# dusk-network/plonk_gadgets

Measured on AMD Instinct MI355X. Metric: gadget constraints/sec (range_check 256-bit), higher is better.
Workload: dtype u64x4 (BLS12-381 scalar, Montgomery limbs); 1 GPU; C2: 2^20 witnesses/GPU x (allocate + range_check(min=0,max=2^254)), n=255, 1031 rows + 1034 vars per witness; items_per_gpu=1048576, items_per_launch=1048576

## Files before the change

plonk_gadgets_amd/csrc/capi.hip:

```cpp
#include "../../include/plonk_gadgets_hip.h"

#include <hip/hip_runtime.h>

#include <algorithm>
#include <cstdio>
#include <cstdlib>
#include <cstring>
#include <initializer_list>
#include <new>
#include <functional>
#include <string>
#include <type_traits>
#include <utility>
#include <vector>

#include "emit.hpp"
#include "fr.hpp"
#include "range_gadgets.hpp"
#include "scalar_gadgets.hpp"
#include "composer.hpp"
#include "permutation.hpp"
#include "materialize.hpp"
#include "permutation_product.hpp"
#include "ntt.hpp"
// ... 17 lines not shown

#define PG_HIP_TRY(expr)                                                                \
    do {                                                                                \
        hipError_t _e = (expr);                                                         \
        if (_e != hipSuccess)                                                           \
            return fail(PG_ERR_HIP, std::string(#expr) + ": " + hipGetErrorString(_e)); \
    } while (0)

#define PG_TRY(expr)                   \
    do {                               \
        pg_status _s = (expr);         \
        if (_s != PG_OK) return _s;    \
    } while (0)

inline pg::Fr to_fr(const pg_scalar *s) {
    pg::Fr f;
    std::memcpy(f.l, s->l, sizeof f.l);
    return f;
}
inline void from_fr(const pg::Fr &f, pg_scalar *out) { std::memcpy(out->l, f.l, sizeof f.l); }

inline bool aligned(const void *p, size_t a) { return (reinterpret_cast<uintptr_t>(p) & (a - 1)) == 0; }

bool is_reduced(const pg::Fr &f) {
    const uint64_t Q[4] = {PG_Q0, PG_Q1, PG_Q2, PG_Q3};
    for (int i = 3; i >= 0; i--) {
        if (f.l[i] < Q[i]) return true;
        if (f.l[i] > Q[i]) return false;
    }
    return false;
}

pg_status check_columns(const pg_columns *c) {
    if (!c) return fail(PG_ERR_INVALID_ARGUMENT, "columns is NULL");
    const void *sc[6] = {c->q_m, c->q_l, c->q_r, c->q_o, c->q_c, c->var_values};
    for (const void *p : sc)
        if (!p || !aligned(p, 16)) return fail(PG_ERR_INVALID_ARGUMENT, "scalar column NULL or not 16-byte aligned");
    const void *wc[3] = {c->w_l, c->w_r, c->w_o};
    for (const void *p : wc)
        if (!p || !aligned(p, 8)) return fail(PG_ERR_INVALID_ARGUMENT, "wire column NULL or not 8-byte aligned");
    return PG_OK;
}

pg_status check_scalars(const void *p, const char *what) {
    if (!p || !aligned(p, 16)) return fail(PG_ERR_INVALID_ARGUMENT, std::string(what) + " NULL or not 16-byte aligned");
    return PG_OK;
}
pg_status check_u64s(const void *p, const char *what, bool nullable = false) {
    if (!p && nullable) return PG_OK;
    if (!p || !aligned(p, 8)) return fail(PG_ERR_INVALID_ARGUMENT, std::string(what) + " NULL or not 8-byte aligned");
    return PG_OK;
}

}

struct pg_engine {
    int device = -1;
    int num_cus = 0;
    uint4 *d_pow2 = nullptr;
    uint32_t *d_rows = nullptr, *d_vars = nullptr;
    uint64_t *d_blk_rows = nullptr, *d_blk_vars = nullptr;
    unsigned long long *d_blk_agg = nullptr;
    uint32_t *d_err_count = nullptr;
    uint64_t scratch_items = 0, scratch_blocks = 0;
    using PlanResult = pg::PlanTotals;
    PlanResult *h_plan = nullptr;
    uint4 *d_prefix = nullptr;
    uint64_t inv_elems = 0;
    hipStream_t side = nullptr;
    hipEvent_t ev_fork = nullptr, ev_inv = nullptr;
    hipStream_t last_stream = nullptr;
    bool have_last = false;
    hipEvent_t ev_switch = nullptr;
    uint4 *d_pp = nullptr;
    uint64_t pp_units = 0;
    uint4 *d_ntt = nullptr;
    uint64_t ntt_units = 0;
    uint4 *d_quot = nullptr, *d_eval = nullptr;
    uint64_t quot_units = 0, eval_units = 0;
    uint4 *d_msm = nullptr, *d_srs = nullptr;
    uint64_t msm_units = 0, srs_units = 0;
    uint4 *d_open = nullptr;
    uint64_t open_units = 0;
};

namespace {

pg_status ensure_scratch(pg_engine *e, uint64_t batch) {
    if (batch <= e->scratch_items && e->d_err_count) return PG_OK;
    PG_HIP_TRY(hipSetDevice(e->device));
    if (e->d_rows) { (void)hipFree(e->d_rows); e->d_rows = nullptr; }
    if (e->d_vars) { (void)hipFree(e->d_vars); e->d_vars = nullptr; }
    if (e->d_blk_rows) { (void)hipFree(e->d_blk_rows); e->d_blk_rows = nullptr; }
    if (e->d_blk_vars) { (void)hipFree(e->d_blk_vars); e->d_blk_vars = nullptr; }
    if (e->d_blk_agg) { (void)hipFree(e->d_blk_agg); e->d_blk_agg = nullptr; }
    e->scratch_items = 0;
    const uint64_t items = batch < 1024 ? 1024 : batch;
    const uint64_t nblk = std::max<uint64_t>((items + pg::kScanBlock - 1) / pg::kScanBlock, 2048);
    PG_HIP_TRY(hipMalloc(&e->d_rows, items * sizeof(uint32_t)));
    PG_HIP_TRY(hipMalloc(&e->d_vars, items * sizeof(uint32_t)));
    PG_HIP_TRY(hipMalloc(&e->d_blk_rows, nblk * sizeof(uint64_t)));
    PG_HIP_TRY(hipMalloc(&e->d_blk_vars, nblk * sizeof(uint64_t)));
    PG_HIP_TRY(hipMalloc(&e->d_blk_agg, (nblk + 1) * sizeof(unsigned long long)));
    PG_HIP_TRY(hipMemset(e->d_blk_agg, 0, (nblk + 1) * sizeof(unsigned long long)));
    e->scratch_blocks = nblk;
    if (!e->d_err_count) {
        PG_HIP_TRY(hipMalloc(&e->d_err_count, sizeof(uint32_t)));
        PG_HIP_TRY(hipMemset(e->d_err_count, 0, sizeof(uint32_t)));
    }
    e->scratch_items = items;
    return PG_OK;
}

pg::PlanScan plan_scan(pg_engine *e, uint64_t batch, uint64_t *d_row_off, uint64_t *d_var_off, bool with_errs) {
    const uint64_t nblk = (batch + pg::kScanBlock - 1) / pg::kScanBlock;
    pg::PlanScan P{};
    P.agg = e->d_blk_agg;
    P.blocks_cap = (uint32_t)e->scratch_blocks;
    P.blk_rows = e->d_blk_rows;
    P.blk_vars = e->d_blk_vars;
    P.row_off = d_row_off;
    P.var_off = d_var_off;
    P.host = e->h_plan;
    P.err_count = with_errs ? e->d_err_count : nullptr;
#if defined(PG_PLAN_TWO_LAUNCHES)
    P.fused = 0;
#else
    P.fused = nblk <= pg::kPlanFusedBlocks ? 1u : 0u;
#endif
    return P;
}

pg_status plan_totals(pg_engine *e, uint64_t *n_rows, uint64_t *n_vars) {
    if (e->h_plan->pad) {
        e->h_plan->pad = 0;
        return fail(PG_ERR_HIP, "a plan's look-back gave up waiting for another block's totals");
    }
    *n_rows = e->h_plan->n_gates;
    *n_vars = e->h_plan->n_vars;
    return PG_OK;
}

pg_status scan_counts(pg_engine *e, uint64_t batch, uint64_t *d_row_off, uint64_t *d_var_off, uint64_t *n_rows,
                      uint64_t *n_vars, hipStream_t st, bool with_errs) {
    const uint32_t nblk = (uint32_t)((batch + pg::kScanBlock - 1) / pg::kScanBlock);
    if (!plan_scan(e, batch, d_row_off, d_var_off, with_errs).fused) {
        const uint32_t prefixed = nblk > pg::kScanDirectBlocks ? 1u : 0u;
        if (prefixed)
            hipLaunchKernelGGL(pg::scan_top_kernel, dim3(1), dim3(pg::kThreads), 0, st, e->d_blk_rows, e->d_blk_vars, nblk);
        hipLaunchKernelGGL(pg::scan_final_kernel, dim3(nblk), dim3(pg::kThreads), 0, st, e->d_rows, e->d_vars, batch,
                           e->d_blk_rows, e->d_blk_vars, d_row_off, d_var_off, prefixed, e->h_plan, with_errs ? e->d_err_count : nullptr);
        PG_HIP_TRY(hipGetLastError());
    }
    if (n_rows) {
        PG_HIP_TRY(hipStreamSynchronize(st));
        PG_TRY(plan_totals(e, n_rows, n_vars));
    }
    return PG_OK;
}

pg::EmitOut make_out(const pg_columns *c, uint64_t batch, int W, uint64_t gate_base, uint64_t var_base, uint64_t zero_var,
                     const uint64_t *row_off, const uint64_t *var_off) {
    pg::EmitOut O;
    O.q[0] = reinterpret_cast<uint4 *>(c->q_m);
    O.q[1] = reinterpret_cast<uint4 *>(c->q_l);
    O.q[2] = reinterpret_cast<uint4 *>(c->q_r);
// ... 1313 lines not shown
```

plonk_gadgets_amd/csrc/capi_composer.inc:

```

struct pg_composer {
    pg_engine *e = nullptr;
    hipStream_t stream = nullptr;
    uint64_t gate_cap = 0, var_cap = 0, n = 0, nvars = 0, zero_var = 0;
    pg::ComposerCols cols{};
    uint64_t *d_stage = nullptr;
    std::vector<uint64_t> pi_gate;
    std::vector<pg_scalar> pi_val;
    std::vector<pg::FourthWire> fourth;
    std::vector<pg::PermSeg> segs;
    void *perm_small = nullptr, *perm_big = nullptr, *val_ws = nullptr;
    void *perm_pieces = nullptr;
    size_t perm_pieces_bytes = 0;
    size_t perm_small_bytes = 0, perm_big_bytes = 0, val_ws_bytes = 0;
    std::vector<void *> ragged;
    uint64_t *h_total = nullptr;
    uint64_t perm_last_sparse = 0;
    uint64_t sparse_hint = 0;
    uint64_t sparse_cap_first = 0;
    bool auto_grow = false;
    uint64_t col_stride = 0;
    void *block = nullptr;
    struct Queued {
        uint8_t kind;
// ... 1509 lines not shown
    const uint32_t grid = (uint32_t)c->e->num_cus * 32;
    pg::MaterializeOut M{};
    pg_scalar *const consts[7] = {out->q_4, out->q_arith, out->q_range, out->q_logic, out->q_fixed_group_add,
                                  out->q_variable_group_add, out->w_4_value};
    for (int k = 0; k < 7; k++) {
        if (!consts[k]) continue;
        PG_TRY(check_scalars(consts[k], "constant column"));
        M.konst[k] = reinterpret_cast<uint4 *>(consts[k]);
    }
    pg_scalar *const vals[3] = {out->w_l_value, out->w_r_value, out->w_o_value};
    for (int i = 0; i < 3; i++) {
        if (!vals[i]) continue;
        PG_TRY(check_scalars(vals[i], "wire value column"));
        M.val[i] = reinterpret_cast<uint4 *>(vals[i]);
    }
    if (out->w_4) {
        PG_TRY(check_u64s(out->w_4, "w_4"));
        M.w_4 = out->w_4;
    }
    const auto generic = [&](uint64_t lo, uint64_t hi) {
        if (hi <= lo) return;
        const uint64_t want = (2 * (hi - lo) + 16383) / 16384;
        hipLaunchKernelGGL(pg::materialize_kernel, dim3((uint32_t)(want < grid ? want : grid)), dim3(pg::kThreads), 0, c->stream, c->cols, M,
                           lo, hi, c->zero_var);
    };
    uint64_t at = 0;
    for (const pg::PermSeg &s : c->segs) {
        if (s.V > pg::kMatWindowVars || s.V == 0 || s.gate_end - s.gate_base < 4096) continue;
        generic(at, s.gate_base);
        uint64_t group = pg::kMatWindowVars / (s.V ? s.V : 1);
        group = group < 1 ? 1 : (group > s.items ? s.items : group);
#ifndef PG_MAT_GRID_PER_CU
#define PG_MAT_GRID_PER_CU 64
#endif
        const uint64_t n_groups = (s.items + group - 1) / group, most = (uint64_t)c->e->num_cus * PG_MAT_GRID_PER_CU;
        const dim3 mgrid((uint32_t)(n_groups < most ? n_groups : most));
        const bool closed = s.wire_kind != pg::WIRES_UNKNOWN && !s.row_off && (pg::ladder_foreign_per_item(s.wire_kind) == 0 || group <= pg::kMatWitItems);
#define PG_MAT_LAUNCH(MODE, KIND)                                                                                                          \
    hipLaunchKernelGGL((pg::materialize_items_kernel<MODE, KIND>), mgrid, dim3(pg::kMatThreads), 0, c->stream, c->cols, M, s, (uint32_t)group, \
                       c->zero_var)
        if (s.row_off && s.wire_kind == pg::WIRES_MAX_BOUND && group <= pg::kMatWitItems)
            hipLaunchKernelGGL((pg::materialize_items_kernel<pg::MAT_SELF, pg::WIRES_MAX_BOUND, true>), mgrid, dim3(pg::kMatThreads), 0, c->stream,
                               c->cols, M, s, (uint32_t)group, c->zero_var);
        else if (s.row_off && s.wire_kind == pg::WIRES_MIX && group < 127)
            hipLaunchKernelGGL((pg::materialize_items_kernel<pg::MAT_SELF, pg::WIRES_MIX, true>), mgrid, dim3(pg::kMatThreads), 0, c->stream,
                               c->cols, M, s, (uint32_t)group, c->zero_var);
        else if (!closed) PG_MAT_LAUNCH(pg::MAT_READ_WIRES, pg::WIRES_UNKNOWN);
        else if (s.wire_kind == pg::WIRES_RANGE_CHECK) PG_MAT_LAUNCH(pg::MAT_SELF, pg::WIRES_RANGE_CHECK);
        else if (s.wire_kind == pg::WIRES_MAX_BOUND) PG_MAT_LAUNCH(pg::MAT_SELF, pg::WIRES_MAX_BOUND);
        else if (s.wire_kind == pg::WIRES_RANGE_CHECK_ALLOCATED) PG_MAT_LAUNCH(pg::MAT_SELF, pg::WIRES_RANGE_CHECK_ALLOCATED);
        else if (s.wire_kind == pg::WIRES_MAX_BOUND_ALLOCATED) PG_MAT_LAUNCH(pg::MAT_SELF, pg::WIRES_MAX_BOUND_ALLOCATED);
        else if (s.wire_kind == pg::WIRES_DECOMPOSITION) PG_MAT_LAUNCH(pg::MAT_SELF, pg::WIRES_DECOMPOSITION);
        else if (s.wire_kind == pg::WIRES_MIX) PG_MAT_LAUNCH(pg::MAT_SELF, pg::WIRES_MIX);
        else PG_MAT_LAUNCH(pg::MAT_READ_WIRES, pg::WIRES_UNKNOWN);
#undef PG_MAT_LAUNCH
        at = s.gate_end;
    }
    generic(at, c->n);
    CallBuffers B(c->stream);
    uint64_t *d_gate; uint4 *d_val; pg::FourthWire *d_fw;
    PG_TRY(upload_sparse(c, B, &d_gate, &d_val, &d_fw));
    if (d_fw)
        hipLaunchKernelGGL(pg::patch_fourth_kernel, dim3(1), dim3(64), 0, c->stream, reinterpret_cast<uint4 *>(out->q_4), out->w_4,
                           reinterpret_cast<uint4 *>(out->w_4_value), c->cols.vars, d_fw, (uint32_t)c->fourth.size());
    PG_HIP_TRY(hipGetLastError());
    PG_HIP_TRY(hipStreamSynchronize(c->stream));
    return PG_OK;
}

#ifndef PG_PERM_LDS_PAD
#define PG_PERM_LDS_PAD 0
#endif
static pg_status perm_reserve(pg_composer *c, void **buf, size_t *have, size_t bytes) {
    if (bytes <= *have) return PG_OK;
    PG_HIP_TRY(hipStreamSynchronize(c->stream));
    if (*buf) (void)hipFree(*buf);
    *buf = nullptr;
    *have = 0;
    PG_HIP_TRY(hipMalloc(buf, bytes));
    *have = bytes;
    return PG_OK;
}

pg_status pg_composer_permutation_reserve(pg_composer *c, uint64_t sparse_positions) {
    if (!c) return fail(PG_ERR_INVALID_ARGUMENT, "composer is NULL");
    c->sparse_cap_first = sparse_positions;
    if (sparse_positions) c->perm_last_sparse = 0;
    return PG_OK;
}

pg_status pg_composer_permutation(pg_composer *c, uint64_t padded_n, uint64_t *d_sigma) {
    if (!c) return fail(PG_ERR_INVALID_ARGUMENT, "composer is NULL");
    PG_TRY(flush(c));
    PG_TRY(check_u64s(d_sigma, "d_sigma"));
    if (padded_n < c->n) return fail(PG_ERR_INVALID_ARGUMENT, "padded_n is smaller than the circuit");
    PG_HIP_TRY(hipSetDevice(c->e->device));
    const uint32_t grid = (uint32_t)c->e->num_cus * 32;
    if (!c->h_total) PG_HIP_TRY(hipHostMalloc(reinterpret_cast<void **>(&c->h_total), 32, hipHostMallocDefault));
    uint32_t pos_bits = 2, var_bits = 1;
    while ((1ull << pos_bits) < 4 * c->n) pos_bits++;
    while ((1ull << var_bits) < c->nvars + 1) var_bits++;
    if (pos_bits + var_bits > 64) return fail(PG_ERR_INVALID_ARGUMENT, "circuit too large for 64-bit (Variable, position) keys");
    std::vector<pg::PermSeg> segs;
    std::vector<std::pair<uint64_t, uint64_t>> gaps;
    uint64_t at = 0, gap_rows = 0;
    for (pg::PermSeg s : c->segs) {
        const auto fits = [&](uint64_t k) {
            return 4 * k * s.L < pg::kPermDone && k * s.V < pg::kPermNone &&
                   pg::perm_local_lds_bytes((uint32_t)(k * s.L), (uint32_t)(k * s.V)) <= pg::kPermLocalLdsLimit;
        };
        if (!fits(1)) continue;
        uint64_t k = 1024 / s.L;
        k = k < 1 ? 1 : (k > s.items ? s.items : k);
        while (k > 1 && !fits(k)) k--;
        const bool closed_ladder = s.wire_kind != pg::WIRES_UNKNOWN && s.wire_kind < pg::WIRES_MIX && (s.row_off ? s.wire_kind == pg::WIRES_MAX_BOUND && s.tail == 0 : s.wire_n >= 2);
        if (closed_ladder || (pg::is_template_kind(s.wire_kind) && s.tail == 0)) k = 1;
        s.group = (uint32_t)k;
        if (s.gate_base > at) gaps.emplace_back(at, s.gate_base);
        segs.push_back(s);
        at = s.gate_end;
    }
    if (c->n > at) gaps.emplace_back(at, c->n);
    for (const auto &g : gaps) gap_rows += g.second - g.first;
    const size_t seg_bytes = (segs.size() * sizeof(pg::PermSeg) + 255) / 256 * 256;
    const size_t fw_bytes = (c->fourth.size() * sizeof(pg::FourthWire) + 255) / 256 * 256;
    PG_TRY(perm_reserve(c, &c->perm_small, &c->perm_small_bytes, seg_bytes + fw_bytes + 256));
    char *small = static_cast<char *>(c->perm_small);
    pg::PermCtx X;
    X.C = c->cols; X.n = c->n; X.padded_n = padded_n; X.zero_var = c->zero_var;
    X.segs = reinterpret_cast<const pg::PermSeg *>(small); X.n_segs = (uint32_t)segs.size();
    X.fw = reinterpret_cast<const pg::FourthWire *>(small + seg_bytes); X.n_fw = (uint32_t)c->fourth.size();
    X.fw_lo = 0; X.fw_span = 0; X.pos_bits = pos_bits;
    X.hole_key = pos_bits + var_bits >= 64 ? ~0ull : (1ull << (pos_bits + var_bits)) - 1;
    if (!c->fourth.empty()) {
        uint64_t lo = ~0ull, hi = 0;
        for (const pg::FourthWire &f : c->fourth) { lo = f.gate < lo ? f.gate : lo; hi = f.gate > hi ? f.gate : hi; }
        X.fw_lo = lo; X.fw_span = hi - lo;
    }
    uint64_t reserved = 0;
    for (pg::PermSeg &s : segs)
        if (s.wire_kind != pg::WIRES_UNKNOWN && !s.row_off && s.wire_n >= 2) {
            s.sparse_base = reserved;
            reserved += s.items * pg::ladder_foreign_per_item(s.wire_kind);
        } else if (pg::is_template_kind(s.wire_kind) && s.tail == 0) {
            s.sparse_base = reserved;
            reserved += s.items * pg::template_foreign_per_item(s.wire_kind);
        }
    const auto ragged_ladder = [](const pg::PermSeg &s) { return s.row_off && s.wire_kind == pg::WIRES_MAX_BOUND && s.tail == 0; };
    const auto template_seg = [](const pg::PermSeg &s) { return pg::is_template_kind(s.wire_kind) && s.tail == 0; };
    const auto needs_pieces = [&](const pg::PermSeg &s) { return ragged_ladder(s) || (template_seg(s) && s.row_off); };
    const auto pieces_of = [](const pg::PermSeg &s) { return (s.gate_end - (s.gate_base & ~1ull) + pg::kPermLadderRows - 1) / pg::kPermLadderRows; };
    {
        uint64_t total_pieces = 0;
        for (const pg::PermSeg &s : segs)
            if (needs_pieces(s)) total_pieces += pieces_of(s);
        if (total_pieces) {
            PG_TRY(perm_reserve(c, &c->perm_pieces, &c->perm_pieces_bytes, total_pieces * sizeof(uint32_t)));
            uint32_t *at_piece = static_cast<uint32_t *>(c->perm_pieces);
            for (pg::PermSeg &s : segs)
                if (needs_pieces(s)) {
                    s.piece_item = at_piece;
                    at_piece += pieces_of(s);
                    const uint64_t want = (s.items + pg::kThreads - 1) / pg::kThreads;
                    hipLaunchKernelGGL(pg::perm_piece_items_kernel, dim3((uint32_t)(want < grid ? want : grid)), dim3(pg::kThreads), 0, c->stream, s,
                                       pg::kPermLadderRows, at_piece - pieces_of(s));
                }
            PG_HIP_TRY(hipGetLastError());
        }
    }
    unsigned long long *d_count = reinterpret_cast<unsigned long long *>(small + seg_bytes + fw_bytes);
    if (!segs.empty())
        PG_HIP_TRY(hipMemcpyAsync(small, segs.data(), segs.size() * sizeof(pg::PermSeg), hipMemcpyHostToDevice, c->stream));
    if (!c->fourth.empty())
        PG_HIP_TRY(hipMemcpyAsync(small + seg_bytes, c->fourth.data(), c->fourth.size() * sizeof(pg::FourthWire),
                                  hipMemcpyHostToDevice, c->stream));
    uint64_t cap = c->sparse_cap_first ? c->sparse_cap_first : 4 * gap_rows + c->sparse_hint + (1ull << 16), nS = 0;
    if (cap < c->perm_last_sparse) cap = c->perm_last_sparse;
    uint64_t *k0 = nullptr, *k1 = nullptr, holes = 0;
    size_t tmp_bytes = 0;
    for (int attempt = 0;; attempt++) {
        uint64_t *nul = nullptr;
        PG_HIP_TRY(rocprim::radix_sort_keys(nullptr, tmp_bytes, nul, nul, (size_t)cap, 0u, pos_bits + var_bits, c->stream));
        const size_t kb = (cap * 8 + 255) / 256 * 256;
        PG_TRY(perm_reserve(c, &c->perm_big, &c->perm_big_bytes, 2 * kb + tmp_bytes + 256));
        k0 = reinterpret_cast<uint64_t *>(c->perm_big);
        k1 = reinterpret_cast<uint64_t *>(static_cast<char *>(c->perm_big) + kb);
        const pg::PermSparse Q{k0, d_count, cap};
        hipLaunchKernelGGL(pg::perm_count_init_kernel, dim3(1), dim3(1), 0, c->stream, d_count, reserved);
        for (const pg::PermSeg &s : segs) {
            const uint64_t groups = (s.items + s.group - 1) / s.group, most = (uint64_t)c->e->num_cus * 64;
            if (s.wire_kind != pg::WIRES_UNKNOWN && !s.row_off && s.wire_n >= 2) {
                const uint64_t pieces = (s.gate_end - (s.gate_base & ~1ull) + pg::kPermLadderRows - 1) / pg::kPermLadderRows;
                const uint64_t lmost = pg::kPermLadderRows <= 2048 ? 0x7fffffffull : most;
                if (pg::kPermLadderLds)
                    PG_HIP_TRY(hipFuncSetAttribute(reinterpret_cast<const void *>(pg::perm_ladder_kernel<false>), hipFuncAttributeMaxDynamicSharedMemorySize,
                                                   (int)pg::kPermLadderLds));
                const uint32_t lds = pg::ladder_foreign_per_item(s.wire_kind) ? 0u : pg::kPermLadderLds;
                hipLaunchKernelGGL(pg::perm_ladder_kernel<false>, dim3((uint32_t)(pieces < lmost ? pieces : lmost)), dim3(pg::kThreads), lds,
                                   c->stream, X, s, Q, d_sigma);
                continue;
            }
            if (template_seg(s)) {
                const uint64_t pieces = pieces_of(s);
                if (pieces > 0x7fffffffull) return fail(PG_ERR_INVALID_ARGUMENT, "segment too large for one launch");
                const uint32_t lds = pg::template_foreign_per_item(s.wire_kind) ? 0u : pg::kPermLadderLds - 8192;
                const pg::TemplateRows T = pg::template_rows(s.wire_kind);
                if (s.row_off) {
                    PG_HIP_TRY(hipFuncSetAttribute(reinterpret_cast<const void *>(pg::perm_template_kernel<true>),
                                                   hipFuncAttributeMaxDynamicSharedMemorySize, (int)pg::kPermLadderLds));
                    hipLaunchKernelGGL(pg::perm_template_kernel<true>, dim3((uint32_t)pieces), dim3(pg::kThreads), lds, c->stream, X, s, T, Q, d_sigma);
                } else {
                    PG_HIP_TRY(hipFuncSetAttribute(reinterpret_cast<const void *>(pg::perm_template_kernel<false>),
                                                   hipFuncAttributeMaxDynamicSharedMemorySize, (int)pg::kPermLadderLds));
                    hipLaunchKernelGGL(pg::perm_template_kernel<false>, dim3((uint32_t)pieces), dim3(pg::kThreads), lds, c->stream, X, s, T, Q, d_sigma);
                }
                continue;
            }
            if (ragged_ladder(s)) {
                const uint64_t pieces = pieces_of(s);
                if (pieces > 0x7fffffffull) return fail(PG_ERR_INVALID_ARGUMENT, "segment too large for one launch");
                if (pg::kPermLadderLds)
                    PG_HIP_TRY(hipFuncSetAttribute(reinterpret_cast<const void *>(pg::perm_ladder_kernel<true>), hipFuncAttributeMaxDynamicSharedMemorySize,
                                                   (int)pg::kPermLadderLds));
                hipLaunchKernelGGL(pg::perm_ladder_kernel<true>, dim3((uint32_t)pieces), dim3(pg::kThreads), pg::kPermLadderLds, c->stream, X, s, Q,
                                   d_sigma);
                continue;
            }
            hipLaunchKernelGGL(pg::perm_item_kernel, dim3((uint32_t)(groups < most ? groups : most)), dim3(pg::kThreads),
                               pg::perm_local_lds_bytes(s.group * s.L, s.group * s.V) + PG_PERM_LDS_PAD, c->stream, X, s, groups, Q, d_sigma);
        }
        for (const auto &g : gaps) {
            const uint64_t nblk = (g.second - g.first + pg::kPermChunk - 1) / pg::kPermChunk;
            hipLaunchKernelGGL(pg::perm_gap_kernel, dim3((uint32_t)nblk), dim3(pg::kThreads), 0, c->stream, X, g.first, g.second, Q,
                               d_sigma);
        }
        PG_HIP_TRY(hipMemcpyAsync(c->h_total, d_count, 16, hipMemcpyDeviceToHost, c->stream));
        PG_HIP_TRY(hipStreamSynchronize(c->stream));
        nS = c->h_total[0];
        holes = c->h_total[1];
        c->perm_last_sparse = nS;
        if (nS <= cap) break;
        if (attempt) return fail(PG_ERR_HIP, "sparse position list grew between two passes");
        cap = nS;
    }
    if (nS) {
        PG_HIP_TRY(rocprim::radix_sort_keys(static_cast<char *>(c->perm_big) + 2 * ((cap * 8 + 255) / 256 * 256), tmp_bytes, k0, k1,
                                            (size_t)nS, 0u, pos_bits + var_bits, c->stream));
        nS -= holes;
    }
    if (nS) {
        const uint64_t want = (nS + pg::kThreads - 1) / pg::kThreads;
        hipLaunchKernelGGL(pg::perm_sparse_link_kernel, dim3((uint32_t)(want < grid ? want : grid)), dim3(pg::kThreads), 0, c->stream,
                           X, k1, nS, d_sigma);
        if (!segs.empty()) {
            const uint64_t wantw = (nS + 255) / 256;
            hipLaunchKernelGGL(pg::perm_splice_kernel, dim3((uint32_t)(wantw < grid ? wantw : grid)), dim3(pg::kThreads), 0, c->stream,
                               X, k1, nS, d_sigma);
        }
    }
    if (padded_n > c->n) {
        const uint64_t per_run = ((padded_n - c->n) / 2 + 1 + pg::kPermIdentityUnits - 1) / pg::kPermIdentityUnits;
        if (4 * per_run > 0x7fffffffull) return fail(PG_ERR_INVALID_ARGUMENT, "padding too large for one launch");
        PG_HIP_TRY(hipFuncSetAttribute(reinterpret_cast<const void *>(pg::perm_identity_kernel), hipFuncAttributeMaxDynamicSharedMemorySize,
                                       (int)pg::kPermIdentityLds));
        hipLaunchKernelGGL(pg::perm_identity_kernel, dim3((uint32_t)(4 * per_run)), dim3(pg::kThreads), pg::kPermIdentityLds, c->stream,
                           d_sigma, c->n, padded_n);
    }
    PG_HIP_TRY(hipGetLastError());
    return PG_OK;
}

pg_status pg_check_rows(pg_engine *e, const pg_columns *cols, uint64_t n_gates, uint64_t var_base, uint64_t n_vars,
                        pg_variable zero_var, int64_t *first_bad, void *stream) {
    if (!e || !first_bad) return fail(PG_ERR_INVALID_ARGUMENT, "NULL argument");
    *first_bad = -1;
    if (n_gates == 0) return PG_OK;
    PG_TRY(check_columns(cols));
    PG_HIP_TRY(hipSetDevice(e->device));
    hipStream_t st = static_cast<hipStream_t>(stream);
    pg::ComposerCols C;
    C.q[0] = reinterpret_cast<uint4 *>(cols->q_m); C.q[1] = reinterpret_cast<uint4 *>(cols->q_l);
    C.q[2] = reinterpret_cast<uint4 *>(cols->q_r); C.q[3] = reinterpret_cast<uint4 *>(cols->q_o);
    C.q[4] = reinterpret_cast<uint4 *>(cols->q_c);
    C.w[0] = cols->w_l; C.w[1] = cols->w_r; C.w[2] = cols->w_o;
    C.vars = reinterpret_cast<uint4 *>(cols->var_values);
    unsigned long long *d_bad = nullptr, h_bad = ~0ull;
    PG_HIP_TRY(hipMalloc(&d_bad, 8));
    PG_HIP_TRY(hipMemcpyAsync(d_bad, &h_bad, 8, hipMemcpyHostToDevice, st));
    hipLaunchKernelGGL(pg::check_kernel, dim3((uint32_t)e->num_cus * 16), dim3(pg::kThreads), 0, st, C, n_gates, var_base, n_vars,
                       zero_var, (const uint64_t *)nullptr, (const uint4 *)nullptr, 0u, (const pg::FourthWire *)nullptr, 0u, d_bad);
    hipError_t le = hipGetLastError();
    if (le == hipSuccess) le = hipMemcpyAsync(&h_bad, d_bad, 8, hipMemcpyDeviceToHost, st);
    if (le == hipSuccess) le = hipStreamSynchronize(st);
    (void)hipFree(d_bad);
    if (le != hipSuccess) return fail(PG_ERR_HIP, std::string("pg_check_rows: ") + hipGetErrorString(le));
    *first_bad = h_bad == ~0ull ? -1 : (int64_t)h_bad;
    return PG_OK;
}

}
```

plonk_gadgets_amd/csrc/permutation.hpp:

```cpp
#pragma once

#include <cstring>

#include <rocprim/rocprim.hpp>

#include "composer.hpp"
#include "range_gadgets.hpp"

namespace pg {

struct PermSeg {
    uint64_t gate_base, gate_end, var_base, var_end;
    uint32_t L, V;
    uint64_t items;
    const uint64_t *row_off, *var_off;
    uint32_t group;
    uint32_t wire_kind, wire_n;
    uint64_t sparse_base;
    uint32_t tail;
    const uint32_t *piece_item;
};
enum : uint32_t { WIRES_UNKNOWN = 0, WIRES_RANGE_CHECK = 1, WIRES_MAX_BOUND = 2, WIRES_RANGE_CHECK_ALLOCATED = 3, WIRES_MAX_BOUND_ALLOCATED = 4,
                  WIRES_DECOMPOSITION = 5,
                  WIRES_MIX = 6,
// ... 302 lines not shown
        return 3;
    }
    if (jj == 1) {
        w2[0] = 1; w2[1] = 2; j2[2] = 3; w2[2] = 1;
        return 0;
    }
    if (jj == 2 * n + 2) {
        j2[0] = 2 * n + 1; w2[0] = 2; j2[2] = 2 * n + 3; w2[2] = 1;
        return 2;
    }
    if (jj == 2 * n + 3) {
        j2[1] = 2 * n + 4; w2[1] = 1; j2[2] = 2 * n + 4; w2[2] = 0;
        return 0;
    }
    w2[1] = 2; j2[2] = 2 * n + 2; w2[2] = 2;
    return 1;
}
__device__ __forceinline__ uint32_t ladder_row(uint32_t kind, uint32_t n, uint32_t j, uint32_t j2[3], uint32_t w2[3], uint32_t tail = 0) {
    const uint32_t L = 2 * n + 5;
    const bool rc = kind == WIRES_RANGE_CHECK || kind == WIRES_RANGE_CHECK_ALLOCATED;
    const uint32_t own = rc ? 2 * L + 1 : L;
    if (tail && j >= own) {
        j2[0] = j; w2[0] = 1; j2[1] = j; w2[1] = 2;
        if (j + 1 < own + tail) { j2[2] = j + 1; w2[2] = 0; }
        else { j2[2] = rc ? 2 * L : 2 * n + 3; w2[2] = 2; }
        return 0;
    }
    if (kind == WIRES_RANGE_CHECK || kind == WIRES_RANGE_CHECK_ALLOCATED) {
        if (j == 2 * L) {
            j2[0] = 2 * n + 3; w2[0] = 2; j2[1] = L + 2 * n + 3; w2[1] = 2; j2[2] = tail ? j + 1 : j; w2[2] = tail ? 0 : 2;
            return 0;
        }
        const uint32_t blk = j >= L ? 1u : 0u, base = blk * L, jj = j - base;
        const uint32_t open = ladder_block_row(jj, n, j2, w2);
#pragma unroll
        for (int w = 0; w < 3; w++) j2[w] += base;
        if (jj == 0) {
            if (kind == WIRES_RANGE_CHECK_ALLOCATED) return 3;
            j2[0] = j; w2[0] = 1; j2[1] = blk ? 0 : L; w2[1] = 0;
        } else if (open == 2) { j2[1] = base; w2[1] = 2; }
        else if (open == 1) { j2[0] = 2 * L; w2[0] = blk; }
        return 0;
    }
    if (kind == WIRES_DECOMPOSITION) {
        const uint32_t open = ladder_block_row(j + 1, n, j2, w2);
#pragma unroll
        for (int w = 0; w < 3; w++) j2[w] -= 1;
        if (open == 2) return 2;
        if (open == 1) { j2[0] = 2 * n + 2; w2[0] = 2; }
        return 0;
    }
    const uint32_t open = ladder_block_row(j, n, j2, w2);
    if (j == 0) {
        if (kind == WIRES_MAX_BOUND_ALLOCATED) return 3;
        j2[0] = 0; w2[0] = 1; j2[1] = 0; w2[1] = 0;
    } else if (open == 2) { j2[1] = 0; w2[1] = 2; }
    else if (open == 1) { j2[0] = tail ? L : 2 * n + 3; w2[0] = tail ? 0 : 2; }
    return 0;
}

__device__ __forceinline__ uint32_t ladder_foreign_wires(uint32_t kind, uint32_t n, uint32_t j) {
    if (kind == WIRES_RANGE_CHECK_ALLOCATED) return j == 0 || j == 2 * n + 5 ? 3u : 0u;
    if (kind == WIRES_MAX_BOUND_ALLOCATED) return j == 0 ? 3u : 0u;
    if (kind == WIRES_DECOMPOSITION) return j == 2 * n + 1 ? 2u : 0u;
    return 0u;
}

__host__ __device__ inline uint32_t ladder_foreign_per_item(uint32_t kind) {
    return kind == WIRES_RANGE_CHECK_ALLOCATED ? 4u : kind == WIRES_MAX_BOUND_ALLOCATED ? 2u : kind == WIRES_DECOMPOSITION ? 1u : 0u;
}
__device__ __forceinline__ uint32_t ladder_foreign_rank(uint32_t kind, uint32_t j, uint32_t w) {
    if (kind == WIRES_DECOMPOSITION) return 0u;
    return (j ? 2u : 0u) + w;
}

#ifndef PG_PERM_LADDER_ROWS
#define PG_PERM_LADDER_ROWS 512
#endif
#ifndef PG_PERM_LADDER_LDS
#define PG_PERM_LADDER_LDS 39936
#endif
constexpr uint32_t kPermLadderRows = PG_PERM_LADDER_ROWS;
constexpr uint32_t kPermLadderLds = PG_PERM_LADDER_LDS;
constexpr uint32_t kPermRaggedWindow = 64;
__global__ __launch_bounds__(kThreads) void perm_piece_items_kernel(const PermSeg S, uint32_t rows_per_piece, uint32_t *piece_item) {
    const uint64_t d = S.gate_base & 1;
    for (uint64_t i = (uint64_t)blockIdx.x * kThreads + threadIdx.x; i < S.items; i += (uint64_t)gridDim.x * kThreads) {
        const uint64_t r0 = S.row_off[i], r1 = S.row_off[i + 1];
        if (i == 0) piece_item[0] = 0;
        for (uint64_t p = (r0 + d + rows_per_piece - 1) / rows_per_piece; p * rows_per_piece < r1 + d; p++)
            if (p) piece_item[p] = (uint32_t)i;
    }
}

template <bool RAGGED>
__global__ __launch_bounds__(kThreads) void perm_ladder_kernel(const PermCtx X, const PermSeg S, const PermSparse Q, uint64_t *sigma) {
    extern __shared__ uint4 perm_ladder_pad[];
    __shared__ uint32_t s_off[RAGGED ? kPermRaggedWindow : 1];
    static_assert(!RAGGED || kPermLadderRows / 9 + 3 <= kPermRaggedWindow, "a piece's items fit the window of prefix sums");
    const uint32_t lane = threadIdx.x & 63, kind = S.wire_kind;
    uint32_t n = S.wire_n;
    if (X.padded_n == 1) perm_ladder_pad[threadIdx.x] = make_uint4(0, 0, 0, 0);
    const uint64_t first = S.gate_base & ~1ull, total = S.gate_end - first;
    const bool wide = (reinterpret_cast<uintptr_t>(sigma) & 15) == 0 && !(X.padded_n & 1);
    const uint32_t recip = (uint32_t)(((1ull << 32) + S.L - 1) / S.L);
    const bool pow2 = (X.padded_n & (X.padded_n - 1)) == 0;
    const uint32_t sh = 63u - (uint32_t)__clzll((long long)X.padded_n);
    auto enc = [&](uint64_t gate, uint32_t wire) { return pow2 ? ((uint64_t)wire << sh) + gate : perm_encode(gate, wire, X.padded_n); };
    auto zero_wires = [&](uint64_t g, uint32_t j) {
        uint32_t z = 0;
        for (uint32_t m = ladder_foreign_wires(kind, n, j); m; m &= m - 1) {
            const uint32_t w = (uint32_t)__ffs((int)m) - 1;
            if (X.C.w[w][g] == X.zero_var) z |= 1u << w;
        }
        return z;
    };
    for (uint64_t base = (uint64_t)blockIdx.x * kPermLadderRows; base < total; base += (uint64_t)gridDim.x * kPermLadderRows) {
        const uint64_t g_first = first + base, rel = g_first < S.gate_base ? 0 : g_first - S.gate_base;
        uint64_t item0, rows0 = 0;
        if constexpr (RAGGED) {
            item0 = S.piece_item[base / kPermLadderRows];
            rows0 = S.row_off[item0];
            __syncthreads();
            if (threadIdx.x < kPermRaggedWindow) {
                const uint64_t i = item0 + threadIdx.x < S.items ? item0 + threadIdx.x : S.items;
                s_off[threadIdx.x] = (uint32_t)(S.row_off[i] - rows0);
            }
            __syncthreads();
        } else {
            item0 = rel / S.L;
            rows0 = item0 * S.L;
        }
        const uint32_t j0 = (uint32_t)(rel - rows0), skip = (uint32_t)(g_first < S.gate_base ? S.gate_base - g_first : 0);
        for (uint32_t t = 2 * threadIdx.x; t < kPermLadderRows; t += 2 * kThreads) {
            uint64_t out[4][2], fitem[2] = {0, 0};
            uint32_t foreign[2] = {0, 0}, fslots[2] = {0, 0}, fj[2] = {0, 0};
            bool live[2];
#pragma unroll
            for (uint32_t h = 0; h < 2; h++) {
                const uint64_t g = g_first + t + h;
                live[h] = g >= S.gate_base && g < S.gate_end;
                const uint32_t tt = t + h - skip;
                uint32_t q, j;
                uint64_t g_item;
#pragma unroll
                for (uint32_t w = 0; w < 4; w++) out[w][h] = 0;
                if constexpr (RAGGED) {
                    if (!live[h]) continue;
                    const uint32_t x = j0 + tt;
                    uint32_t lo = 0;
#pragma unroll
                    for (uint32_t step = kPermRaggedWindow / 2; step; step >>= 1)
                        if (s_off[lo + step] <= x) lo += step;
                    q = lo;
                    j = x - s_off[lo];
                    n = (s_off[lo + 1] - s_off[lo] - 5) >> 1;
                    g_item = S.gate_base + rows0 + s_off[lo];
                } else {
                    q = __umulhi(j0 + tt, recip);
                    j = (j0 + tt) - q * S.L;
                    g_item = S.gate_base + (item0 + q) * S.L;
                }
                if (!live[h]) continue;
                uint32_t j2[3], w2[3];
                const uint32_t fw = ladder_row(kind, n, j, j2, w2, S.tail), zw = fw ? zero_wires(g, j) : 0u;
                foreign[h] = fw & ~zw;
                fslots[h] = fw;
                fitem[h] = item0 + q;
                fj[h] = j;
#pragma unroll
                for (uint32_t w = 0; w < 3; w++) {
                    if (fw >> w & 1) {
                        const uint32_t later = (zw | 8u) & ~((2u << w) - 1);
                        out[w][h] = enc(g, (uint32_t)__ffs((int)later) - 1);
                    } else {
                        out[w][h] = enc(g_item + j2[w], w2[w]);
                    }
                }
                if (g + 1 < S.gate_end) {
                    const uint32_t jn = j + 1 == S.L ? 0 : j + 1;
                    const uint32_t zn = ladder_foreign_wires(kind, n, jn) ? zero_wires(g + 1, jn) : 0u;
                    out[3][h] = enc(g + 1, (uint32_t)__ffs((int)(zn | 8u)) - 1);
                } else {
                    out[3][h] = perm_next_zero_from(X, S.gate_end);
                }
            }
            const uint64_t g = g_first + t;
#pragma unroll
            for (uint32_t w = 0; w < 4; w++) {
                const bool skip0 = !live[0] || (foreign[0] >> w & 1), skip1 = !live[1] || (foreign[1] >> w & 1);
                uint64_t *dst = sigma + enc(g, w);
                if (wide && !skip0 && !skip1)
                    store16(reinterpret_cast<uint4 *>(dst), make_uint4((uint32_t)out[w][0], (uint32_t)(out[w][0] >> 32), (uint32_t)out[w][1],
                                                                      (uint32_t)(out[w][1] >> 32)));
                else {
                    if (!skip0) dst[0] = out[w][0];
                    if (!skip1) dst[1] = out[w][1];
                }
            }
            if (fslots[0] | fslots[1]) {
                const uint32_t F = ladder_foreign_per_item(kind);
#pragma unroll
                for (uint32_t h = 0; h < 2; h++)
                    for (uint32_t m = fslots[h]; m; m &= m - 1) {
                        const uint32_t w = (uint32_t)__ffs((int)m) - 1;
                        const uint64_t at = S.sparse_base + fitem[h] * F + ladder_foreign_rank(kind, fj[h], w);
                        if (foreign[h] >> w & 1) perm_sparse_put(X, Q, at, X.C.w[w][g + h], g + h, w);
                        else {
                            if (at < Q.cap) Q.keys[at] = X.hole_key;
                            atomicAdd(Q.count + 1, 1ull);
                        }
                    }
            }
        }
    }
}

constexpr uint8_t kTmplForeign = 0xF0, kTmplZero = 0xFE, kTmplNone = 0xFF;
constexpr uint32_t kTmplRows = 10;
struct SegTemplate {
    uint8_t L[2], V[2];
    uint8_t wire[2][kTmplRows][3];
};
#define PG_T3(a, b, c) {a, b, c}
#define PG_TF0 0xF0
#define PG_TF1 0xF1
#define PG_TF2 0xF2
#define PG_TZ 0xFE
#define PG_TX PG_T3(0xFF, 0xFF, 0xFF)
constexpr SegTemplate kSegTemplates[WIRES_KINDS - WIRES_MIX] = {
    {{10, 8}, {15, 13},
     {{PG_T3(0, 5, PG_TZ), PG_T3(7, 7, 7), PG_T3(0, 6, 7), PG_T3(8, 8, 8), PG_T3(1, 2, 9), PG_T3(8, 2, 10), PG_T3(9, 10, 11), PG_T3(3, 4, 12),
       PG_T3(13, 12, 14), PG_T3(14, 12, 12)},
      {PG_T3(0, 5, PG_TZ), PG_T3(6, 6, 6), PG_T3(1, 2, 7), PG_T3(6, 2, 8), PG_T3(7, 8, 9), PG_T3(3, 4, 10), PG_T3(11, 10, 12), PG_T3(12, 10, 10),
       PG_TX, PG_TX}}},
    {{1, 0}, {1, 0}, {{PG_T3(PG_TF0, PG_TF1, 0), PG_TX, PG_TX, PG_TX, PG_TX, PG_TX, PG_TX, PG_TX, PG_TX, PG_TX}, {PG_TX, PG_TX, PG_TX, PG_TX, PG_TX, PG_TX, PG_TX, PG_TX, PG_TX, PG_TX}}},
    {{4, 0}, {4, 0}, {{PG_T3(0, 0, 0), PG_T3(PG_TF0, PG_TF1, 1), PG_T3(0, PG_TF1, 2), PG_T3(1, 2, 3), PG_TX, PG_TX, PG_TX, PG_TX, PG_TX, PG_TX}, {PG_TX, PG_TX, PG_TX, PG_TX, PG_TX, PG_TX, PG_TX, PG_TX, PG_TX, PG_TX}}},
    {{3, 0}, {3, 0}, {{PG_T3(PG_TF0, PG_TF1, 0), PG_T3(1, 0, 2), PG_T3(2, 0, 0), PG_TX, PG_TX, PG_TX, PG_TX, PG_TX, PG_TX, PG_TX}, {PG_TX, PG_TX, PG_TX, PG_TX, PG_TX, PG_TX, PG_TX, PG_TX, PG_TX, PG_TX}}},
    {{3, 1}, {3, 1}, {{PG_T3(PG_TF0, 0, PG_TZ), PG_T3(2, 2, 2), PG_T3(PG_TF0, 1, 2), PG_TX, PG_TX, PG_TX, PG_TX, PG_TX, PG_TX, PG_TX}, {PG_T3(PG_TF0, 0, PG_TZ), PG_TX, PG_TX, PG_TX, PG_TX, PG_TX, PG_TX, PG_TX, PG_TX, PG_TX}}},
    {{1, 0}, {1, 0}, {{PG_T3(PG_TF0, PG_TF1, 0), PG_TX, PG_TX, PG_TX, PG_TX, PG_TX, PG_TX, PG_TX, PG_TX, PG_TX}, {PG_TX, PG_TX, PG_TX, PG_TX, PG_TX, PG_TX, PG_TX, PG_TX, PG_TX, PG_TX}}},
    {{1, 0}, {0, 0}, {{PG_T3(PG_TF0, PG_TF1, PG_TF2), PG_TX, PG_TX, PG_TX, PG_TX, PG_TX, PG_TX, PG_TX, PG_TX, PG_TX}, {PG_TX, PG_TX, PG_TX, PG_TX, PG_TX, PG_TX, PG_TX, PG_TX, PG_TX, PG_TX}}},
};
#undef PG_T3
#undef PG_TF0
#undef PG_TF1
#undef PG_TF2
#undef PG_TZ
#undef PG_TX
__host__ __device__ inline uint32_t template_foreign_per_item(uint32_t kind) {
    return kind == WIRES_SELECT_ZERO || kind == WIRES_MAYBE_EQUAL || kind == WIRES_IS_NON_ZERO || kind == WIRES_GATE_OUT ? 2u
           : kind == WIRES_SELECT_ONE || kind == WIRES_GATE_ROWS ? 3u : 0u;
}
__host__ __device__ inline bool is_template_kind(uint32_t kind) { return kind >= WIRES_MIX && kind < WIRES_KINDS; }

struct TemplateRows {
    uint64_t row[2][kTmplRows];
    uint8_t L[2], V[2], F[2];
    uint8_t Fmax, pad;
};
inline TemplateRows template_rows(uint32_t kind) {
    const SegTemplate &T = kSegTemplates[kind - WIRES_MIX];
    TemplateRows R{};
    for (uint32_t sh = 0; sh < 2; sh++) {
        R.L[sh] = T.L[sh];
        R.V[sh] = T.V[sh];
        uint32_t foreign = 0;
        const uint32_t n = (uint32_t)T.L[sh] * 3;
        for (uint32_t p = 0; p < n; p++) {
            const uint8_t code = T.wire[sh][p / 3][p % 3];
            uint64_t b = 0;
            if (code < kTmplForeign) {
                uint32_t first = 0xff, next = 0xff;
                for (uint32_t q = 0; q < n; q++)
                    if (T.wire[sh][q / 3][q % 3] == code) {
                        if (first == 0xff) first = q;
                        if (q > p && next == 0xff) next = q;
                    }
                const uint32_t z = next != 0xff ? next : first;
                b = 1u | (uint64_t)code << 2 | (uint64_t)(4 * (z / 3) + z % 3) << 6;
            } else if (code < kTmplZero) {
                b = 2u | (uint64_t)foreign++ << 12;
            } else if (code == kTmplZero) {
                b = 3u;
            }
            R.row[sh][p / 3] |= b << (16 * (p % 3));
        }
        R.F[sh] = (uint8_t)foreign;
    }
    R.Fmax = (uint8_t)template_foreign_per_item(kind);
    return R;
}

constexpr uint32_t kTmplWindow = 1024;
template <bool RAGGED>
__global__ __launch_bounds__(kThreads) void perm_template_kernel(const PermCtx X, const PermSeg S, const TemplateRows T, const PermSparse Q,
                                                                uint64_t *sigma) {
    extern __shared__ uint4 perm_template_pad[];
    __shared__ uint64_t s_row[2][kTmplRows];
    __shared__ uint32_t s_off[RAGGED ? kTmplWindow : 1];
    static_assert(kPermLadderRows + 3 <= kTmplWindow, "a piece's items fit the window of prefix sums");
    if (X.padded_n == 1) perm_template_pad[threadIdx.x] = make_uint4(0, 0, 0, 0);
    const uint32_t Lf = T.L[0], Ls = T.L[1], Fmax = T.Fmax, Ff = T.F[0], Fs = T.F[1];
    if (threadIdx.x < 2 * kTmplRows) s_row[threadIdx.x / kTmplRows][threadIdx.x % kTmplRows] = T.row[threadIdx.x / kTmplRows][threadIdx.x % kTmplRows];
    __syncthreads();
    const uint64_t first = S.gate_base & ~1ull, total = S.gate_end - first;
    const bool wide = (reinterpret_cast<uintptr_t>(sigma) & 15) == 0 && !(X.padded_n & 1);
    const uint32_t recip = (uint32_t)(((1ull << 32) + Lf - 1) / Lf);
    const bool pow2 = (X.padded_n & (X.padded_n - 1)) == 0;
    const uint32_t sh_bits = 63u - (uint32_t)__clzll((long long)X.padded_n);
    auto enc = [&](uint64_t gate, uint32_t wire) { return pow2 ? ((uint64_t)wire << sh_bits) + gate : perm_encode(gate, wire, X.padded_n); };
    for (uint64_t base = (uint64_t)blockIdx.x * kPermLadderRows; base < total; base += (uint64_t)gridDim.x * kPermLadderRows) {
        const uint64_t g_first = first + base, rel = g_first < S.gate_base ? 0 : g_first - S.gate_base;
        uint64_t item0, rows0;
        if constexpr (RAGGED) {
            item0 = S.piece_item[base / kPermLadderRows];
            rows0 = S.row_off[item0];
            __syncthreads();
            for (uint32_t e = threadIdx.x; e < kTmplWindow; e += kThreads) {
                const uint64_t i = item0 + e < S.items ? item0 + e : S.items;
                s_off[e] = (uint32_t)(S.row_off[i] - rows0);
            }
            __syncthreads();
        } else {
            item0 = rel / Lf;
            rows0 = item0 * Lf;
        }
        const uint32_t j0 = (uint32_t)(rel - rows0), skip = (uint32_t)(g_first < S.gate_base ? S.gate_base - g_first : 0);
        struct Row { uint32_t item, j, sh, rows; uint64_t g_item, word; };
        auto locate = [&](uint32_t x, Row &R) {
            if constexpr (RAGGED) {
                uint32_t lo = 0;
#pragma unroll
                for (uint32_t step = kTmplWindow / 2; step; step >>= 1)
                    if (s_off[lo + step] <= x) lo += step;
                R.item = lo;
                R.j = x - s_off[lo];
                R.rows = s_off[lo + 1] - s_off[lo];
                R.sh = R.rows == Lf ? 0u : 1u;
                R.g_item = S.gate_base + rows0 + s_off[lo];
            } else {
                R.item = Lf == 1 ? x : __umulhi(x, recip);
                R.j = x - R.item * Lf;
                R.sh = 0;
                R.rows = Lf;
                R.g_item = S.gate_base + rows0 + (uint64_t)R.item * Lf;
            }
            R.word = s_row[R.sh][R.j];
        };
        auto step = [&](Row &R) {
            if (R.j + 1 < R.rows) R.j++;
            else {
                R.g_item += R.rows;
                R.item++;
                R.j = 0;
                if constexpr (RAGGED) {
                    R.rows = s_off[R.item + 1] - s_off[R.item];
                    R.sh = R.rows == Lf ? 0u : 1u;
                }
            }
            R.word = s_row[R.sh][R.j];
        };
        auto zero_mask = [&](uint64_t g, uint64_t word) {
            uint32_t z = 0;
#pragma unroll
            for (uint32_t w = 0; w < 3; w++) {
                const uint32_t type = (uint32_t)(word >> (16 * w)) & 3u;
                if (type == 3u) z |= 1u << w;
                else if (type == 2u && X.C.w[w][g] == X.zero_var) z |= 1u << w;
            }
            return z;
        };
        for (uint32_t t = 2 * threadIdx.x; t < kPermLadderRows; t += 2 * kThreads) {
            uint64_t out[4][2];
            uint32_t keep[2] = {0, 0};
            bool live[3];
            Row R[3];
// ... 162 lines not shown
```

Measured before the change: 32.77 billion constraints/s.

## Add wave-uniform interior fast path to permutation ladder kernel and hoist attribute setup

Adds a fast path to the permutation ladder kernel for range-check and max-bound wires. When a whole wave of rows lies in the interior of an item, the sigma outputs are computed directly from a closed-form pattern, skipping the per-row item search and wiring logic. Other changes: the ragged window search runs once per row pair, sigma addresses use precomputed column offsets instead of enc(), ragged blocks process a single piece, and hipFuncSetAttribute calls are done once per engine. This adds complexity and correctness risk at interior boundaries and for the ragged window sizing.

```diff
diff --git a/plonk_gadgets_amd/csrc/capi.hip b/plonk_gadgets_amd/csrc/capi.hip
--- a/plonk_gadgets_amd/csrc/capi.hip
+++ b/plonk_gadgets_amd/csrc/capi.hip
@@ -123,6 +123,7 @@
     uint64_t msm_units = 0, srs_units = 0;
     uint4 *d_open = nullptr;
     uint64_t open_units = 0;
+    bool perm_attributes_set = false;
 };
 
 namespace {
diff --git a/plonk_gadgets_amd/csrc/capi_composer.inc b/plonk_gadgets_amd/csrc/capi_composer.inc
--- a/plonk_gadgets_amd/csrc/capi_composer.inc
+++ b/plonk_gadgets_amd/csrc/capi_composer.inc
@@ -1615,6 +1615,20 @@
     return PG_OK;
 }
 
+static pg_status perm_kernel_attributes(pg_engine *e) {
+    if (e->perm_attributes_set) return PG_OK;
+    const auto raise = [](const void *kernel, uint32_t bytes) {
+        return bytes ? hipFuncSetAttribute(kernel, hipFuncAttributeMaxDynamicSharedMemorySize, (int)bytes) : hipSuccess;
+    };
+    PG_HIP_TRY(raise(reinterpret_cast<const void *>(pg::perm_ladder_kernel<false>), pg::kPermLadderLds));
+    PG_HIP_TRY(raise(reinterpret_cast<const void *>(pg::perm_ladder_kernel<true>), pg::kPermLadderLds));
+    PG_HIP_TRY(raise(reinterpret_cast<const void *>(pg::perm_template_kernel<false>), pg::kPermLadderLds));
+    PG_HIP_TRY(raise(reinterpret_cast<const void *>(pg::perm_template_kernel<true>), pg::kPermLadderLds));
+    PG_HIP_TRY(raise(reinterpret_cast<const void *>(pg::perm_identity_kernel), pg::kPermIdentityLds));
+    e->perm_attributes_set = true;
+    return PG_OK;
+}
+
 pg_status pg_composer_permutation_reserve(pg_composer *c, uint64_t sparse_positions) {
     if (!c) return fail(PG_ERR_INVALID_ARGUMENT, "composer is NULL");
     c->sparse_cap_first = sparse_positions;
@@ -1628,6 +1642,7 @@
     PG_TRY(check_u64s(d_sigma, "d_sigma"));
     if (padded_n < c->n) return fail(PG_ERR_INVALID_ARGUMENT, "padded_n is smaller than the circuit");
     PG_HIP_TRY(hipSetDevice(c->e->device));
+    PG_TRY(perm_kernel_attributes(c->e));
     const uint32_t grid = (uint32_t)c->e->num_cus * 32;
     if (!c->h_total) PG_HIP_TRY(hipHostMalloc(reinterpret_cast<void **>(&c->h_total), 32, hipHostMallocDefault));
     uint32_t pos_bits = 2, var_bits = 1;
@@ -1725,9 +1740,6 @@
             if (s.wire_kind != pg::WIRES_UNKNOWN && !s.row_off && s.wire_n >= 2) {
                 const uint64_t pieces = (s.gate_end - (s.gate_base & ~1ull) + pg::kPermLadderRows - 1) / pg::kPermLadderRows;
                 const uint64_t lmost = pg::kPermLadderRows <= 2048 ? 0x7fffffffull : most;
-                if (pg::kPermLadderLds)
-                    PG_HIP_TRY(hipFuncSetAttribute(reinterpret_cast<const void *>(pg::perm_ladder_kernel<false>), hipFuncAttributeMaxDynamicSharedMemorySize,
-                                                   (int)pg::kPermLadderLds));
                 const uint32_t lds = pg::ladder_foreign_per_item(s.wire_kind) ? 0u : pg::kPermLadderLds;
                 hipLaunchKernelGGL(pg::perm_ladder_kernel<false>, dim3((uint32_t)(pieces < lmost ? pieces : lmost)), dim3(pg::kThreads), lds,
                                    c->stream, X, s, Q, d_sigma);
@@ -1739,12 +1751,8 @@
                 const uint32_t lds = pg::template_foreign_per_item(s.wire_kind) ? 0u : pg::kPermLadderLds - 8192;
                 const pg::TemplateRows T = pg::template_rows(s.wire_kind);
                 if (s.row_off) {
-                    PG_HIP_TRY(hipFuncSetAttribute(reinterpret_cast<const void *>(pg::perm_template_kernel<true>),
-                                                   hipFuncAttributeMaxDynamicSharedMemorySize, (int)pg::kPermLadderLds));
                     hipLaunchKernelGGL(pg::perm_template_kernel<true>, dim3((uint32_t)pieces), dim3(pg::kThreads), lds, c->stream, X, s, T, Q, d_sigma);
                 } else {
-                    PG_HIP_TRY(hipFuncSetAttribute(reinterpret_cast<const void *>(pg::perm_template_kernel<false>),
-                                                   hipFuncAttributeMaxDynamicSharedMemorySize, (int)pg::kPermLadderLds));
                     hipLaunchKernelGGL(pg::perm_template_kernel<false>, dim3((uint32_t)pieces), dim3(pg::kThreads), lds, c->stream, X, s, T, Q, d_sigma);
                 }
                 continue;
@@ -1752,9 +1760,6 @@
             if (ragged_ladder(s)) {
                 const uint64_t pieces = pieces_of(s);
                 if (pieces > 0x7fffffffull) return fail(PG_ERR_INVALID_ARGUMENT, "segment too large for one launch");
-                if (pg::kPermLadderLds)
-                    PG_HIP_TRY(hipFuncSetAttribute(reinterpret_cast<const void *>(pg::perm_ladder_kernel<true>), hipFuncAttributeMaxDynamicSharedMemorySize,
-                                                   (int)pg::kPermLadderLds));
                 hipLaunchKernelGGL(pg::perm_ladder_kernel<true>, dim3((uint32_t)pieces), dim3(pg::kThreads), pg::kPermLadderLds, c->stream, X, s, Q,
                                    d_sigma);
                 continue;
@@ -1794,8 +1799,6 @@
     if (padded_n > c->n) {
         const uint64_t per_run = ((padded_n - c->n) / 2 + 1 + pg::kPermIdentityUnits - 1) / pg::kPermIdentityUnits;
         if (4 * per_run > 0x7fffffffull) return fail(PG_ERR_INVALID_ARGUMENT, "padding too large for one launch");
-        PG_HIP_TRY(hipFuncSetAttribute(reinterpret_cast<const void *>(pg::perm_identity_kernel), hipFuncAttributeMaxDynamicSharedMemorySize,
-                                       (int)pg::kPermIdentityLds));
         hipLaunchKernelGGL(pg::perm_identity_kernel, dim3((uint32_t)(4 * per_run)), dim3(pg::kThreads), pg::kPermIdentityLds, c->stream,
                            d_sigma, c->n, padded_n);
     }
diff --git a/plonk_gadgets_amd/csrc/permutation.hpp b/plonk_gadgets_amd/csrc/permutation.hpp
--- a/plonk_gadgets_amd/csrc/permutation.hpp
+++ b/plonk_gadgets_amd/csrc/permutation.hpp
@@ -408,7 +408,8 @@
 #endif
 constexpr uint32_t kPermLadderRows = PG_PERM_LADDER_ROWS;
 constexpr uint32_t kPermLadderLds = PG_PERM_LADDER_LDS;
-constexpr uint32_t kPermRaggedWindow = 64;
+constexpr uint32_t kPermWaveRows = 2 * 64;
+constexpr uint32_t kPermRaggedWindow = kPermLadderRows / 9 + 3 <= 64 ? 64 : kPermLadderRows / 9 + 3 <= 128 ? 128 : 256;
 __global__ __launch_bounds__(kThreads) void perm_piece_items_kernel(const PermSeg S, uint32_t rows_per_piece, uint32_t *piece_item) {
     const uint64_t d = S.gate_base & 1;
     for (uint64_t i = (uint64_t)blockIdx.x * kThreads + threadIdx.x; i < S.items; i += (uint64_t)gridDim.x * kThreads) {
@@ -423,7 +424,7 @@
 __global__ __launch_bounds__(kThreads) void perm_ladder_kernel(const PermCtx X, const PermSeg S, const PermSparse Q, uint64_t *sigma) {
     extern __shared__ uint4 perm_ladder_pad[];
     __shared__ uint32_t s_off[RAGGED ? kPermRaggedWindow : 1];
-    static_assert(!RAGGED || kPermLadderRows / 9 + 3 <= kPermRaggedWindow, "a piece's items fit the window of prefix sums");
+    static_assert(kPermLadderRows / 9 + 3 <= kPermRaggedWindow && kPermRaggedWindow <= kThreads, "a piece's items fit the window of prefix sums");
     const uint32_t lane = threadIdx.x & 63, kind = S.wire_kind;
     uint32_t n = S.wire_n;
     if (X.padded_n == 1) perm_ladder_pad[threadIdx.x] = make_uint4(0, 0, 0, 0);
@@ -441,13 +442,13 @@
         }
         return z;
     };
-    for (uint64_t base = (uint64_t)blockIdx.x * kPermLadderRows; base < total; base += (uint64_t)gridDim.x * kPermLadderRows) {
+    const uint64_t col[4] = {0, X.padded_n, 2 * X.padded_n, 3 * X.padded_n};
+    for (uint64_t base = (uint64_t)blockIdx.x * kPermLadderRows; base < total; base += RAGGED ? total : (uint64_t)gridDim.x * kPermLadderRows) {
         const uint64_t g_first = first + base, rel = g_first < S.gate_base ? 0 : g_first - S.gate_base;
         uint64_t item0, rows0 = 0;
         if constexpr (RAGGED) {
             item0 = S.piece_item[base / kPermLadderRows];
             rows0 = S.row_off[item0];
-            __syncthreads();
             if (threadIdx.x < kPermRaggedWindow) {
                 const uint64_t i = item0 + threadIdx.x < S.items ? item0 + threadIdx.x : S.items;
                 s_off[threadIdx.x] = (uint32_t)(S.row_off[i] - rows0);
@@ -463,9 +464,54 @@
             uint32_t foreign[2] = {0, 0}, fslots[2] = {0, 0}, fj[2] = {0, 0};
             bool live[2];
 #pragma unroll
+            for (uint32_t h = 0; h < 2; h++) live[h] = g_first + t + h >= S.gate_base && g_first + t + h < S.gate_end;
+            const uint32_t t0 = __builtin_amdgcn_readfirstlane(t);
+            bool interior = false;
+            uint32_t step0 = 0;
+            if ((kind == WIRES_RANGE_CHECK || kind == WIRES_MAX_BOUND) && g_first + t0 >= S.gate_base && g_first + t0 + kPermWaveRows <= S.gate_end) {
+                const uint32_t x0 = j0 + t0 - skip;
+                uint32_t jf, nn = S.wire_n;
+                if constexpr (RAGGED) {
+                    uint32_t q0 = ~0u;
+#pragma unroll
+                    for (uint32_t e = 0; e < kPermRaggedWindow; e += 64) q0 += (uint32_t)__popcll(__ballot(s_off[e + lane] <= x0));
+                    const uint32_t o0 = __builtin_amdgcn_readfirstlane(s_off[q0]), o1 = __builtin_amdgcn_readfirstlane(s_off[q0 + 1]);
+                    jf = x0 - o0;
+                    nn = (o1 - o0 - 5) >> 1;
+                } else {
+                    jf = x0 - __umulhi(x0, recip) * S.L;
+                }
+                const uint32_t lb = 2 * nn + 5;
+                const uint32_t jjf = kind == WIRES_RANGE_CHECK && jf >= lb ? jf - lb : jf;
+                interior = jjf >= 4 && jjf + kPermWaveRows - 1 <= 2 * nn;
+                step0 = jjf & 1;
+            }
+            if (interior) {
+#pragma unroll
+                for (uint32_t h = 0; h < 2; h++) {
+                    const uint64_t g = g_first + t + h;
+                    const bool step = (step0 ^ h) & 1;
+                    out[0][h] = g + (step ? col[0] - 1 : col[1]);
+                    out[1][h] = g + (step ? col[2] - 2 : col[2]);
+                    out[2][h] = g + (step ? col[1] + 2 : col[0] + 1);
+                    out[3][h] = g + (col[3] + 1);
+                }
+            } else {
+            uint32_t lo2[2] = {0, 0};
+            if constexpr (RAGGED) {
+                if (live[0] || live[1]) {
+                    const uint32_t x = j0 + t - skip + (live[0] ? 0u : 1u);
+                    uint32_t lo = 0;
+#pragma unroll
+                    for (uint32_t step = kPermRaggedWindow / 2; step; step >>= 1)
+                        if (s_off[lo + step] <= x) lo += step;
+                    lo2[0] = lo;
+                    lo2[1] = live[0] && s_off[lo + 1] <= x + 1 ? lo + 1 : lo;
+                }
+            }
+#pragma unroll
             for (uint32_t h = 0; h < 2; h++) {
                 const uint64_t g = g_first + t + h;
-                live[h] = g >= S.gate_base && g < S.gate_end;
                 const uint32_t tt = t + h - skip;
                 uint32_t q, j;
                 uint64_t g_item;
@@ -474,10 +520,7 @@
                 if constexpr (RAGGED) {
                     if (!live[h]) continue;
                     const uint32_t x = j0 + tt;
-                    uint32_t lo = 0;
-#pragma unroll
-                    for (uint32_t step = kPermRaggedWindow / 2; step; step >>= 1)
-                        if (s_off[lo + step] <= x) lo += step;
+                    const uint32_t lo = lo2[h];
                     q = lo;
                     j = x - s_off[lo];
                     n = (s_off[lo + 1] - s_off[lo] - 5) >> 1;
@@ -511,11 +554,12 @@
                     out[3][h] = perm_next_zero_from(X, S.gate_end);
                 }
             }
+            }
             const uint64_t g = g_first + t;
 #pragma unroll
             for (uint32_t w = 0; w < 4; w++) {
                 const bool skip0 = !live[0] || (foreign[0] >> w & 1), skip1 = !live[1] || (foreign[1] >> w & 1);
-                uint64_t *dst = sigma + enc(g, w);
+                uint64_t *dst = sigma + (g + col[w]);
                 if (wide && !skip0 && !skip1)
                     store16(reinterpret_cast<uint4 *>(dst), make_uint4((uint32_t)out[w][0], (uint32_t)(out[w][0] >> 32), (uint32_t)out[w][1],
                                                                       (uint32_t)(out[w][1] >> 32)));
@@ -617,7 +661,7 @@
     return R;
 }
 
-constexpr uint32_t kTmplWindow = 1024;
+constexpr uint32_t kTmplWindow = kPermLadderRows + 3 <= 1024 ? 1024 : kPermLadderRows + 3 <= 2048 ? 2048 : 4096;
 template <bool RAGGED>
 __global__ __launch_bounds__(kThreads) void perm_template_kernel(const PermCtx X, const PermSeg S, const TemplateRows T, const PermSparse Q,
                                                                 uint64_t *sigma) {
```

Result: no change. 32.70 billion constraints/s, median of 2 (-0.2%).
